# etrigger/Parsip

Hardware: AMD Instinct MI355X
Metric: Mcells/sec polygonized, 256^3 grid 32-prim BlobTree, at 1/2/4/8 MI355X (higher is better)
Workload: dtype f32

## Files before the change

### parsip_amd/csrc/psgpu_device.h

```cpp
#pragma once
#include "psgpu_model.h"

namespace psgpu {

typedef const __attribute__((address_space(4))) DevModel* ModelPtr;
typedef const __attribute__((address_space(4))) DevPrim CPrim;
typedef const __attribute__((address_space(4))) DevOp COp;
typedef const __attribute__((address_space(4))) CubeTablesDev* TablePtr;
__device__ __forceinline__ ModelPtr as_const(const DevModel* m) { return (ModelPtr)m; }
__device__ __forceinline__ TablePtr as_const(const CubeTablesDev* t) { return (TablePtr)t; }

__device__ __forceinline__ Instr load_instr(ModelPtr M, int pc) {
    typedef const __attribute__((address_space(4))) uint32_t* CU32;
    const CU32 w = (CU32)(&M->instr[pc]);
    const uint32_t words[3] = {w[0], w[1], w[2]};
    Instr I;
    __builtin_memcpy(&I, words, 12);
    return I;
}

__device__ __forceinline__ float max_ref(float a, float b) { return a > b ? a : b; }
__device__ __forceinline__ float min_ref(float a, float b) { return a < b ? a : b; }
__device__ __forceinline__ float m01(bool c) { return c ? 1.0f : 0.0f; }
__device__ __forceinline__ int lane_id() { return __lane_id(); }
// ... 210 lines not shown
    }
    return wyvill(prim_dist2<TYPE, PR>(P, x, y, z));
}

__device__ __forceinline__ float prim_field(CPrim& P, float pX, float pY, float pZ) {
    float x = pX, y = pY, z = pZ;
    if (P.hasMatrix) {
        x = ((P.mat[0] * pX + P.mat[1] * pY) + P.mat[2] * pZ) + P.mat[3];
        y = ((P.mat[4] * pX + P.mat[5] * pY) + P.mat[6] * pZ) + P.mat[7];
        z = ((P.mat[8] * pX + P.mat[9] * pY) + P.mat[10] * pZ) + P.mat[11];
    }
    float d2;
    switch (P.type) {
    case PSGPU_T_POINT: d2 = prim_dist2<PSGPU_T_POINT, CPrim>(P, x, y, z); break;
    case PSGPU_T_LINE: d2 = prim_dist2<PSGPU_T_LINE, CPrim>(P, x, y, z); break;
    case PSGPU_T_CYLINDER: d2 = prim_dist2<PSGPU_T_CYLINDER, CPrim>(P, x, y, z); break;
    case PSGPU_T_TRIANGLE: d2 = prim_dist2<PSGPU_T_TRIANGLE, CPrim>(P, x, y, z); break;
    case PSGPU_T_CUBE: d2 = prim_dist2<PSGPU_T_CUBE, CPrim>(P, x, y, z); break;
    case PSGPU_T_DISC: d2 = prim_dist2<PSGPU_T_DISC, CPrim>(P, x, y, z); break;
    case PSGPU_T_RING: d2 = prim_dist2<PSGPU_T_RING, CPrim>(P, x, y, z); break;
    default: d2 = 0.0f; break;
    }
    return wyvill(d2);
}

__device__ __forceinline__ float op_field(uint32_t type, float lf, float rf, float resY, float last) {
    switch (type) {
    case PSGPU_T_BLEND: return lf + rf;
    case PSGPU_T_RICCI: {
        const float base = lf + rf;
        float den = resY * base;
        den = resY - den;
        den = base + den;
        return base * (1.0f / den);
    }
    case PSGPU_T_UNION: return max_ref(lf, rf);
    case PSGPU_T_INTERSECT: return min_ref(lf, rf);
    case PSGPU_T_DIF: return min_ref(lf, 1.0f - rf);
    case PSGPU_T_SMOOTHDIF: return lf * (1.0f - rf);
    case 22: case 23: case 24: case 25: return lf;
    default: return last;
    }
}

__device__ __forceinline__ bool op_colour_weights(uint32_t type, float lf, float rf, float v, float* wl, float* wr) {
    switch (type) {
    case PSGPU_T_BLEND: case PSGPU_T_RICCI:
        *wl = 2.0f * (0.5f + lf) - 1.0f;
        *wr = 2.0f * (0.5f + rf) - 1.0f;
        return true;
    case PSGPU_T_UNION: case PSGPU_T_INTERSECT:
        *wl = m01((v - lf) == 0.0f);
        *wr = m01((v - rf) == 0.0f);
        return true;
    case PSGPU_T_DIF: case PSGPU_T_SMOOTHDIF:
        *wl = m01(lf == v);
        *wr = m01((1.0f - rf) == v);
        return true;
    default:
        return false;
    }
}

struct CullMask {
    uint64_t lo, hi;
    uint64_t inLo, inHi;
};
__device__ __forceinline__ bool op_inside(const CullMask& cm, uint32_t k) {
    return k < 64 ? ((cm.inLo >> k) & 1ull) : ((cm.inHi >> (k - 64)) & 1ull);
}

struct CullLanes {
    CullSeg s[2];
    bool two;
};

__device__ __forceinline__ CullSeg load_cullseg(ModelPtr M, int i) {
    typedef const __attribute__((address_space(4))) float* CF;
    const CF f = (CF)(&M->cull[i]);
    CullSeg S;
    S.a[0] = f[0]; S.a[1] = f[1]; S.a[2] = f[2];
    S.u[0] = f[3]; S.u[1] = f[4]; S.u[2] = f[5];
    S.invUU = f[6]; S.radius = f[7];
    S.tmin = f[8]; S.tmax = f[9]; S.axisClear = f[10]; S.pad = f[11];
    return S;
}

__device__ __forceinline__ CullLanes load_cull_lanes(ModelPtr M) {
    CullLanes L;
    L.two = M->ctPrims > 64u;
    L.s[0] = load_cullseg(M, lane_id());
    if (L.two) L.s[1] = load_cullseg(M, 64 + lane_id());
    return L;
}

__device__ __forceinline__ CullMask cull_mask_from(const CullLanes& L, float x0, float y0, float z0, float x1,
                                                   float y1, float z1) {
    CullMask cm{0ull, 0ull};
    float c[3], h;
    if (!cull_box(x0, y0, z0, x1, y1, z1, c, &h)) return cm;
    cm.lo = ballot(cull_one(L.s[0], c[0], c[1], c[2], h));
    if (L.two) cm.hi = ballot(cull_one(L.s[1], c[0], c[1], c[2], h));
    return cm;
}

__device__ __forceinline__ CullMask cull_mask_box(ModelPtr M, float x0, float y0, float z0, float x1, float y1,
                                                  float z1) {
    return cull_mask_from(load_cull_lanes(M), x0, y0, z0, x1, y1, z1);
}

__device__ __forceinline__ CullMask cull_mask_points(const CullLanes& L, float px, float py, float pz, bool enable,
                                                     float ext = 0.0f) {
    if (!enable) return CullMask{0ull, 0ull};
    if (ballot(!(px == px) || !(py == py) || !(pz == pz)) != 0ull) return CullMask{0ull, 0ull};
    return cull_mask_from(L, wave_min(px), wave_min(py), wave_min(pz), wave_max(px) + ext, wave_max(py) + ext,
                          wave_max(pz) + ext);
}
__device__ __forceinline__ CullMask cull_mask_points(ModelPtr M, float px, float py, float pz, bool enable,
                                                     float ext = 0.0f) {
    if (!enable) return CullMask{0ull, 0ull};
    return cull_mask_points(load_cull_lanes(M), px, py, pz, true, ext);
}

__device__ __forceinline__ bool culled(const CullMask& cm, uint32_t i) {
    return i < 64 ? ((cm.lo >> i) & 1ull) : ((cm.hi >> (i - 64)) & 1ull);
}

constexpr float kBoundEps = 2e-4f;

struct BoundBox {
    float cx, cy, cz, h;
    float xs[4], ys[4], zs[4];
};

template <int TYPE, class PR>
__device__ __forceinline__ float prim_true_dist(PR& P, float x, float y, float z, float* axisD) {
    float d2 = 0.0f;
    if (TYPE == PSGPU_T_POINT) {
        const float dx = x - P.pos[0], dy = y - P.pos[1], dz = z - P.pos[2];
        d2 = dx * dx + dy * dy + dz * dz;
    } else if (TYPE == PSGPU_T_LINE) {
        const float ux = P.dir[0] - P.pos[0], uy = P.dir[1] - P.pos[1], uz = P.dir[2] - P.pos[2];
        const float dx = x - P.pos[0], dy = y - P.pos[1], dz = z - P.pos[2];
        const float t = (dx * ux + dy * uy + dz * uz) / (ux * ux + uy * uy + uz * uz);
        const float ex = dx - t * ux, ey = dy - t * uy, ez = dz - t * uz;
        d2 = ex * ex + ey * ey + ez * ez;
    } else if (TYPE == PSGPU_T_CYLINDER) {
        const float px = x - P.pos[0], py = y - P.pos[1], pz = z - P.pos[2];
        float yy = px * P.dir[0] + py * P.dir[1] + pz * P.dir[2];
        const float rr = px * px + py * py + pz * pz - yy * yy;
        const float r = __builtin_amdgcn_sqrtf(rr > 0.0f ? rr : 0.0f);
        *axisD = r;
        const float xx = fmaxf(r - P.res[0], 0.0f);
        yy = yy > 0.0f ? fmaxf(yy - P.res[1], 0.0f) : yy;
        d2 = xx * xx + yy * yy;
    } else if (TYPE == PSGPU_T_CUBE) {
        const float ex = fmaxf(fabsf(x - P.pos[0]) - P.res[0], 0.0f);
        const float ey = fmaxf(fabsf(y - P.pos[1]) - P.res[0], 0.0f);
        const float ez = fmaxf(fabsf(z - P.pos[2]) - P.res[0], 0.0f);
        d2 = ex * ex + ey * ey + ez * ez;
    }
    return __builtin_amdgcn_sqrtf(d2);
}

__device__ __forceinline__ float wyvill_of_dist(float d) {
    const float t = 1.0f - d * d;
    return t > 0.0f ? (t * t) * t : 0.0f;
}

template <int TYPE, class PR>
__device__ __forceinline__ void prim_bound(PR& P, const BoundBox& B, float* lo, float* hi, bool* ok) {
    float axisD = 1e30f;
    const float d = prim_true_dist<TYPE, PR>(P, B.cx, B.cy, B.cz, &axisD);
    if (TYPE == PSGPU_T_CYLINDER) *ok = *ok && (axisD - B.h > 0.05f);
    *hi = wyvill_of_dist(fmaxf(d - B.h, 0.0f)) + kBoundEps;
    *lo = wyvill_of_dist(d + B.h) - kBoundEps;
}

__device__ __forceinline__ void bound_op(uint32_t type, float ll, float lh, float rl, float rh, float* lo, float* hi) {
    switch (type) {
    case PSGPU_T_BLEND: *lo = ll + rl; *hi = lh + rh; break;
    case PSGPU_T_UNION: *lo = fmaxf(ll, rl); *hi = fmaxf(lh, rh); break;
    case PSGPU_T_INTERSECT: *lo = fminf(ll, rl); *hi = fminf(lh, rh); break;
    case PSGPU_T_DIF: *lo = fminf(ll, 1.0f - rh); *hi = fminf(lh, 1.0f - rl); break;
    case PSGPU_T_SMOOTHDIF: {
        const float a = 1.0f - rh, b = 1.0f - rl;
        const float p0 = ll * a, p1 = ll * b, p2 = lh * a, p3 = lh * b;
        *lo = fminf(fminf(p0, p1), fminf(p2, p3));
        *hi = fmaxf(fmaxf(p0, p1), fmaxf(p2, p3));
    } break;
    default: *lo = ll; *hi = lh; break;
    }
}

template <class OR>
__device__ __forceinline__ void bound_prune(OR& b, const BoundBox& B, float* lo, float* hi) {
    bool anyZ = false, allX = true, noX = true, allY = true, noY = true;
#pragma unroll
    for (int i = 0; i < 4; ++i) {
        anyZ = anyZ | ((B.zs[i] >= b.lo[2]) & (b.hi[2] >= B.zs[i]));
        const bool ix = (B.xs[i] >= b.lo[0]) & (b.hi[0] >= B.xs[i]);
        const bool iy = (B.ys[i] >= b.lo[1]) & (b.hi[1] >= B.ys[i]);
        allX = allX & ix; noX = noX & !ix;
        allY = allY & iy; noY = noY & !iy;
    }
    if (!anyZ && noX && noY) {
        *lo = 0.0f;
        *hi = 0.0f;
    } else if (!(anyZ || allX || allY)) {
        *lo = fminf(*lo, 0.0f);
        *hi = fmaxf(*hi, 0.0f);
    }
}

struct InterpEval {
    ModelPtr M;
    float* sl;
    __device__ InterpEval(ModelPtr m, float* slots) : M(m), sl(slots) {}

    template <int GROUP, bool COLOR>
    __device__ __forceinline__ float eval(float px, float py, float pz, const CullMask& cm, float* colOut) const {
        const int n = (int)M->nInstr;
        const bool noOps = M->ctOps == 0;
        int resume = 0;
        float last = 0.0f, acc = 0.0f;
        float lc0 = 0.0f, lc1 = 0.0f, lc2 = 0.0f;
        constexpr int SW = COLOR ? 4 : 1;
        for (int pc = 0; pc < n; ++pc) {
            const Instr I = load_instr(M, pc);
            const bool act = pc >= resume;
            if (I.kind == kEnter) {
                COp& O = M->ops[I.idx];
                bool in = ((px >= O.lo[0]) & (O.hi[0] >= px)) | ((py >= O.lo[1]) & (O.hi[1] >= py)) |
                          ((pz >= O.lo[2]) & (O.hi[2] >= pz));
                bool anyIn = group_any<GROUP>(act && in);
                bool prune = act && !anyIn;
                if (prune) {
                    resume = I.skipTo;
                    sl[(I.out * SW) * 64] = 0.0f;
                    last = 0.0f;
                }
                if (!COLOR) {
                    if (ballot(pc + 1 >= resume) == 0ull) pc = I.skipTo - 1;
                }
            } else if (I.kind == kPrim) {
                if (COLOR) {
                    float f = 0.0f;
                    if (act && !culled(cm, I.idx)) f = prim_field(M->prims[I.idx], px, py, pz);
                    sl[(I.out * SW) * 64] = f;
                } else if (act) {
                    float f = 0.0f;
                    if (!culled(cm, I.idx)) f = prim_field(M->prims[I.idx], px, py, pz);
                    sl[I.out * 64] = f;
                }
            } else if (I.kind == kOp) {
                if (COLOR || act) {
                    const float lf = sl[(I.lslot * SW) * 64];
                    const float rf = sl[(I.rslot * SW) * 64];
                    float v = op_field(I.type, lf, rf, M->ops[I.idx].resY, last);
// ... 91 lines not shown
__device__ __forceinline__ void phase_stamp_after(const Params& p, int ph, uint32_t bit, float dep) {
    if (!PSGPU_FIN_PHASES || !(p.debug & bit) || !p.stamps) return;
    const uint32_t w = blockIdx.x * (blockDim.x >> 6) + (threadIdx.x >> 6);
    if (w >= p.stampCap) return;
    uint64_t t;
    asm volatile("s_memrealtime %0\n\ts_waitcnt lgkmcnt(0)" : "=s"(t) : "v"(dep));
    if (lane_id() == 0) p.stamps[3 * (size_t)kNumStampKernels * p.stampCap + 8 * (size_t)w + ph] = t;
}
__device__ __forceinline__ void span_end(const Params& p, int K, uint64_t t0) {
    const uint64_t t1 = stamp_now();
    if (lane_id() == 0) {
        uint64_t* s = p.spans + 2 * ((size_t)K * kSpanLanes + (blockIdx.x & (kSpanLanes - 1)));
        atomicMin(reinterpret_cast<unsigned long long*>(s), (unsigned long long)t0);
        atomicMax(reinterpret_cast<unsigned long long*>(s + 1), (unsigned long long)t1);
    }
}
__device__ __forceinline__ uint32_t wave_hw_id() {
    const uint32_t hw = (uint32_t)__builtin_amdgcn_s_getreg((31 << 11) | 4);
    const uint32_t xcc = (uint32_t)__builtin_amdgcn_s_getreg((31 << 11) | 20) & 15u;
    return (hw & 0xffffu) | (xcc << 16);
}
__device__ __forceinline__ void mpu_ticks_s1(const Params& p, uint32_t w, uint64_t t0) {
    uint64_t* r = p.mpuTicks + 4 * (size_t)w;
    r[0] = t0;
    r[1] = stamp_now();
    r[2] = 0ull;
    r[3] = (uint64_t)wave_hw_id();
}
__device__ __forceinline__ void mpu_ticks_s2(const Params& p, uint32_t m) {
    const uint64_t t = stamp_now();
    const uint32_t hw = wave_hw_id();
    if (lane_id() == 0) {
        uint64_t* r = p.mpuTicks + 4 * (size_t)(m - p.mpuBegin);
        atomicMax(reinterpret_cast<unsigned long long*>(r + 2), (unsigned long long)t);
        reinterpret_cast<uint32_t*>(r + 3)[1] = hw;
    }
}
#define PSGPU_STAMPED(K, ITEM, CALL)                                             \
    {                                                                             \
        const uint64_t t0_ = (p.stamps || p.spans) ? psgpu::stamp_now() : 0ull;  \
        uint32_t item_ = blockIdx.x * (blockDim.x >> 6) + (threadIdx.x >> 6);     \
        CALL;                                                                     \
        if (K == 1 && p.mpuTicks && ITEM != 0xffffffffu) psgpu::mpu_ticks_s2(p, ITEM); \
        if (p.stamps) psgpu::stamp_end(p, K, t0_, ITEM);                          \
        if (p.spans) psgpu::span_end(p, K, t0_);                                  \
    }

__device__ __forceinline__ void mpu_origin(const Params& p, uint32_t m, float o[3]) {
    uint32_t k, jk;
    const uint32_t i = div_by(m, p.dims[2] * p.dims[1], p.divMagic[1], &jk);
    const uint32_t j = div_by(jk, p.dims[2], p.divMagic[0], &k);
    o[0] = p.lo[0] + (float)i * p.side;
    o[1] = p.lo[1] + (float)j * p.side;
    o[2] = p.lo[2] + (float)k * p.side;
}

__device__ __forceinline__ uint32_t wave_sum(uint32_t v) { return lane_value(wave_incl_scan(v), 63); }


__device__ __forceinline__ uint32_t front_tag(const Params& p) { return p.ctr->epoch + 1u; }

__device__ __forceinline__ void stamp_live_word(const Params& p, bool on, const CullMask& cm, uint64_t above) {
    if (on && p.stamps && lane_id() == 0) {
        const uint32_t w = blockIdx.x * (blockDim.x >> 6) + (threadIdx.x >> 6);
        if (w < p.stampCap)
            p.stamps[3 * (size_t)kNumStampKernels * p.stampCap + 8 * (size_t)w + 7] =
                (uint64_t)(128 - __popcll(cm.lo) - __popcll(cm.hi)) | above;
    }
}

__device__ __forceinline__ BoundBox octant_box(const Params& p, const float o[3], int c) {
    BoundBox B;
#pragma unroll
    for (int i = 0; i < 4; ++i) {
        B.xs[i] = o[0] + (float)(4 * (c & 1) + i) * p.cs;
        B.ys[i] = o[1] + (float)(4 * ((c >> 1) & 1) + i) * p.cs;
        B.zs[i] = o[2] + (float)(4 * (c >> 2) + i) * p.cs;
    }
    const float hx = 0.5f * (B.xs[3] - B.xs[0]), hy = 0.5f * (B.ys[3] - B.ys[0]), hz = 0.5f * (B.zs[3] - B.zs[0]);
    B.cx = 0.5f * (B.xs[0] + B.xs[3]);
    B.cy = 0.5f * (B.ys[0] + B.ys[3]);
    B.cz = 0.5f * (B.zs[0] + B.zs[3]);
    B.h = __builtin_amdgcn_sqrtf(hx * hx + hy * hy + hz * hz) * 1.0001f + 1e-4f;
    return B;
}

__device__ __forceinline__ uint32_t proven_mask(bool ok, float lo, float hi, uint32_t flags8) {
    const uint64_t bOut = ballot(ok && hi < 0.5f), bIn = ballot(ok && lo >= 0.5f);
    uint32_t proven8 = 0;
#pragma unroll
    for (int q = 0; q < 8; ++q) {
        const bool all = ((bOut >> (8 * q)) & 0xffull) == 0xffull || ((bIn >> (8 * q)) & 0xffull) == 0xffull;
        proven8 |= (all ? 1u : 0u) << q;
    }
    return proven8 & flags8;
}

__device__ __forceinline__ CullMask queue_masks(const Params& p, const CullLanes& cl, const float o[3],
                                                uint32_t queue8, uint32_t mOf, int lane) {
    CullMask mine{0ull, 0ull};
    if (!p.cull) return mine;
    const float eg = 7.0f * p.cs + 0.001f;
    ModelPtr Mo = as_const(p.model);
    const uint32_t nOps = p.opInside ? Mo->ctOps : 0u;
    float bl[2][3], bh[2][3];
#pragma unroll
    for (int h = 0; h < 2; ++h) {
        const uint32_t k = 64u * h + (uint32_t)lane;
#pragma unroll
        for (int a = 0; a < 3; ++a) {
            bl[h][a] = k < nOps ? p.model->ops[k].lo[a] : 1.0f;
            bh[h][a] = k < nOps ? p.model->ops[k].hi[a] : -1.0f;
        }
    }
    for (uint32_t qm = queue8; qm != 0u; qm &= qm - 1u) {
        const int q = __builtin_ctz(qm);
        const float ox = __int_as_float(__builtin_amdgcn_readlane(__float_as_int(o[0]), 8 * q));
        const float oy = __int_as_float(__builtin_amdgcn_readlane(__float_as_int(o[1]), 8 * q));
        const float oz = __int_as_float(__builtin_amdgcn_readlane(__float_as_int(o[2]), 8 * q));
        CullMask g = cull_mask_from(cl, ox, oy, oz, ox + eg, oy + eg, oz + eg);
        if (nOps != 0u) g.inLo = ballot((uint32_t)lane < nOps && op_inside_box(bl[0], bh[0], ox, oy, oz, p.cs));
        if (nOps > 64u)
            g.inHi = ballot(64u + (uint32_t)lane < nOps && op_inside_box(bl[1], bh[1], ox, oy, oz, p.cs));
        const uint32_t wq = lane_value(mOf, q) - p.mpuBegin;
        if (lane == 0) {
            p.mpuMasks[4 * wq] = g.lo;
            p.mpuMasks[4 * wq + 1] = g.hi;
            p.mpuMasks[4 * wq + 2] = g.inLo;
            p.mpuMasks[4 * wq + 3] = g.inHi;
        }
        if (lane == q) mine = g;
    }
    return mine;
}

struct QueueEntry {
    uint32_t m;
    CullMask cm;

    template <bool FRONT, class T>
    static __device__ __forceinline__ void put(T* at, T v) {
        if constexpr (FRONT) __hip_atomic_store(at, v, __ATOMIC_RELAXED, __HIP_MEMORY_SCOPE_AGENT);
        else *at = v;
    }
    template <bool FRONT, class T>
    static __device__ __forceinline__ T get(T* at) {
        if constexpr (FRONT) return __hip_atomic_load(at, __ATOMIC_RELAXED, __HIP_MEMORY_SCOPE_AGENT);
        else return *at;
    }
    template <bool FRONT>
    __device__ __forceinline__ void store(const Params& p, uint32_t slotq) const {
        put<FRONT>(&p.pq[slotq], m);
        if (p.cull) {
            put<FRONT>(&p.pqMask[4 * slotq], cm.lo);
            put<FRONT>(&p.pqMask[4 * slotq + 1], cm.hi);
            put<FRONT>(&p.pqMask[4 * slotq + 2], cm.inLo);
            put<FRONT>(&p.pqMask[4 * slotq + 3], cm.inHi);
        }
    }
    static __device__ __forceinline__ void publish(const Params& p, uint32_t slotq, bool mine) {
        asm volatile("s_waitcnt vmcnt(0)" ::: "memory");
        if (mine) put<true>(&p.fqReady[slotq], front_tag(p));
    }
    template <bool FRONT>
    static __device__ __forceinline__ QueueEntry load(const Params& p, ModelPtr M, uint32_t slotq) {
        QueueEntry e{uniform(get<FRONT>(&p.pq[slotq])), CullMask{0ull, 0ull}};
// ... 1116 lines not shown
```

### parsip_amd/csrc/psgpu_host.cpp

```cpp
#include <hip/hip_runtime.h>

#include <atomic>
#include <algorithm>
#include <numeric>
#include <cmath>
#include <cstdio>
#include <cstdlib>
#include <cstring>
#include <ctime>
#include <functional>
#include <limits>
#include <memory>
#include <chrono>
#include <mutex>
#include <string>
#include <thread>
#include <vector>

#include "../../include/parsip_gpu.h"
#include "psgpu_internal.h"
#include "psgpu_launch.h"


using namespace psgpu;
// ... 186 lines not shown
        }
        D.nInstr = P.ctPrims;
        D.nSlots = 1;
    } else {
        ProgramBuilder b(O);
        b.emit(0, 0, 0);
        if (!b.ok) return PSGPU_RET_INVALID_BVH;
        D.nInstr = (uint32_t)b.prog.size();
        std::copy(b.prog.begin(), b.prog.end(), D.instr);
        D.nSlots = (uint32_t)std::max(1, b.maxSlot);
    }
    for (uint32_t i = 0; i < 128; ++i) {
        DevOp& d = D.ops[i];
        d.lo[0] = O.vBoxLoX[i]; d.lo[1] = O.vBoxLoY[i]; d.lo[2] = O.vBoxLoZ[i];
        d.hi[0] = O.vBoxHiX[i]; d.hi[1] = O.vBoxHiY[i]; d.hi[2] = O.vBoxHiZ[i];
        d.resY = O.resY[i];
        d.type = O.opType[i];
    }
    const float* pc[3] = {P.colorX, P.colorY, P.colorZ};
    std::function<void(int)> zero_col = [&](int op) {
        const uint32_t t = O.opType[op], kind = O.opChildKind[op];
        const uint32_t L = O.opLeftChild[op], R = O.opRightChild[op];
        if (kind & 2) zero_col((int)L);
        if (kind & 1) zero_col((int)R);
        float cl[3], cr[3];
        for (int k = 0; k < 3; ++k) {
            cl[k] = (kind & 2) ? D.zeroCol[L][k] : pc[k][L];
            cr[k] = (kind & 1) ? D.zeroCol[R][k] : pc[k][R];
        }
        const float lf = 0.0f, rf = 0.0f;
        float v = 0.0f, wl = 0.0f, wr = 0.0f;
        bool weighted = true;
        switch (t) {
        case PSGPU_OP_BLEND: v = lf + rf; wl = 2.0f * (0.5f + lf) - 1.0f; wr = 2.0f * (0.5f + rf) - 1.0f; break;
        case PSGPU_OP_UNION: v = lf > rf ? lf : rf; wl = (v - lf) == 0.0f ? 1.0f : 0.0f; wr = (v - rf) == 0.0f ? 1.0f : 0.0f; break;
        case PSGPU_OP_INTERSECT: v = lf < rf ? lf : rf; wl = (v - lf) == 0.0f ? 1.0f : 0.0f; wr = (v - rf) == 0.0f ? 1.0f : 0.0f; break;
        case PSGPU_OP_DIF: { const float q = 1.0f - rf; v = lf < q ? lf : q; wl = lf == v ? 1.0f : 0.0f; wr = (1.0f - rf) == v ? 1.0f : 0.0f; } break;
        case PSGPU_OP_SMOOTHDIF: v = lf * (1.0f - rf); wl = lf == v ? 1.0f : 0.0f; wr = (1.0f - rf) == v ? 1.0f : 0.0f; break;
        default: weighted = false; break;
        }
        for (int k = 0; k < 3; ++k) {
            if (weighted) D.zeroCol[op][k] = wl * cl[k] + wr * cr[k];
            else if (t >= PSGPU_OP_WARPTWIST && t <= PSGPU_OP_WARPSHEAR) D.zeroCol[op][k] = cl[k];
            else D.zeroCol[op][k] = 0.0f;
        }
    };
    if (O.ctOps > 0) zero_col(0);
    for (uint32_t i = 0; i < 128; ++i) {
        DevPrim& d = D.prims[i];
        d.pos[0] = P.posX[i]; d.pos[1] = P.posY[i]; d.pos[2] = P.posZ[i];
        d.dir[0] = P.dirX[i]; d.dir[1] = P.dirY[i]; d.dir[2] = P.dirZ[i];
        d.res[0] = P.resX[i]; d.res[1] = P.resY[i]; d.res[2] = P.resZ[i];
        d.col[0] = P.colorX[i]; d.col[1] = P.colorY[i]; d.col[2] = P.colorZ[i];
        d.type = P.skeletType[i];
        const uint32_t im = P.idxMatrix[i];
        d.hasMatrix = im != 0;
        if (im != 0) {
            if (im >= 128) return PSGPU_RET_PARAM_ERROR;
            memcpy(d.mat, &Mx.matrix[im * PSGPU_PRIM_MATRIX_STRIDE], 12 * sizeof(float));
        }
        bool c = !d.hasMatrix && finite3(d.pos);
        switch (d.type) {
        case PSGPU_PRIM_POINT: break;
        case PSGPU_PRIM_LINE: {
            const double ux = (double)d.dir[0] - d.pos[0], uy = (double)d.dir[1] - d.pos[1],
                         uz = (double)d.dir[2] - d.pos[2];
            c = c && finite3(d.dir) && (ux * ux + uy * uy + uz * uz) > 1e-6;
        } break;
        case PSGPU_PRIM_CUBE: c = c && std::isfinite(d.res[0]) && d.res[0] >= 0.0f; break;
        case PSGPU_PRIM_CYLINDER: {
            const double n2 = (double)d.dir[0] * d.dir[0] + (double)d.dir[1] * d.dir[1] + (double)d.dir[2] * d.dir[2];
            c = c && finite3(d.dir) && std::fabs(n2 - 1.0) < 1e-4 && d.res[0] >= 0.0f && d.res[1] >= 0.0f &&
                std::isfinite(d.res[0]) && std::isfinite(d.res[1]);
        } break;
        default: c = false; break;
        }
        CullSeg& cs = D.cull[i];
        memset(&cs, 0, sizeof(cs));
        const float inf = std::numeric_limits<float>::infinity();
        cs.radius = inf;
        cs.tmin = 0.0f;
        cs.tmax = 1.0f;
        cs.axisClear = -inf;
        uint32_t flags = c ? 1u : 0u;
        if (c) {
            for (int a = 0; a < 3; ++a) cs.a[a] = d.pos[a];
            cs.radius = 0.0f;
            double uu = 0.0;
            if (d.type == PSGPU_PRIM_LINE) {
                for (int a = 0; a < 3; ++a) cs.u[a] = d.dir[a] - d.pos[a];
                cs.tmin = -inf;
                cs.tmax = inf;
                flags |= 2u;
            } else if (d.type == PSGPU_PRIM_CYLINDER) {
                for (int a = 0; a < 3; ++a) cs.u[a] = d.res[1] * d.dir[a];
                cs.radius = d.res[0];
                cs.axisClear = 0.05f;
                flags |= 4u;
            } else if (d.type == PSGPU_PRIM_CUBE) {
                cs.radius = (float)(d.res[0] * 1.7320508075688772 * (1.0 + 1e-6));
            }
            for (int a = 0; a < 3; ++a) uu += (double)cs.u[a] * cs.u[a];
            cs.invUU = uu > 0.0 ? (float)(1.0 / uu) : 0.0f;
            if (d.type == PSGPU_PRIM_CYLINDER && uu == 0.0) {
                flags &= ~1u;
                cs.radius = inf;
            }
        } else if (d.type == PSGPU_PRIM_TRIANGLE) {
            cs.radius = -inf;
        }
        if (i >= P.ctPrims) cs.radius = inf;
        d.cullable = flags;
    }
    bool bnd = D.nInstr > 0;
    for (uint32_t k = 0; k < D.nInstr; ++k) {
        const Instr& I = D.instr[k];
        if (I.kind == kOp && !((I.type >= 14 && I.type <= 18) || (I.type >= 22 && I.type <= 25))) bnd = false;
        if (I.kind == kPrim || I.kind == kSumPrim) {
            const DevPrim& q = D.prims[I.idx];
            if (!(q.type == PSGPU_PRIM_TRIANGLE || (q.cullable & 1u))) bnd = false;
        }
    }
    D.boundable = bnd ? 1u : 0u;
    D.rootZeroValid = root_zero_set(D, D.rootZero) ? 1u : 0u;
    if (!D.rootZeroValid) D.rootZero[0] = D.rootZero[1] = 0ull;
    return PSGPU_RET_SUCCESS;
}

void lattice_dims(float cs, const PsVec3f& lo, const PsVec3f& hi, uint32_t d[3]) {
    const float ext[3] = {hi.x - lo.x, hi.y - lo.y, hi.z - lo.z};
    for (int a = 0; a < 3; ++a) {
        const float q = ext[a] / cs;
        const int cells = (int)std::ceil(q);
        int n = cells / PSGPU_CELLS_PER_MPU;
        if (cells % PSGPU_CELLS_PER_MPU != 0) ++n;
        d[a] = n > 0 ? (uint32_t)n : 0u;
    }
}

const char* kKernelNames[kNumKernels] = {"k_precheck", "k_mpu", "k_vertex", "k_finish"};

}

namespace psgpu {
int hip_fail(hipError_t e, const char* what) {
    if (e == hipSuccess) return PSGPU_RET_SUCCESS;
    fprintf(stderr, "psgpu: %s failed: %s\n", what, hipGetErrorString(e));
    return e == hipErrorOutOfMemory ? PSGPU_RET_NOT_ENOUGH_MEM : PSGPU_RET_DEVICE_ERROR;
}

int set_device(psgpu_ctx* c) { return hip_fail(hipSetDevice(c->device), "hipSetDevice"); }
}

namespace {

void brick_layout(const psgpu_ctx* c, uint32_t* i0, uint32_t bd[3]) {
    const uint32_t nyz = c->dims[1] * c->dims[2];
    const uint32_t first = nyz ? c->mpuBegin / nyz : 0;
    const uint32_t last = (nyz && c->mpuCount) ? (c->mpuBegin + c->mpuCount - 1) / nyz : first;
    *i0 = first / 2;
    bd[0] = c->mpuCount ? last / 2 - first / 2 + 1 : 0;
    bd[1] = (c->dims[1] + 1) / 2;
    bd[2] = (c->dims[2] + 1) / 2;
}
uint32_t brick_stride(uint32_t n, bool spread) {
    if (!spread || n < 3) return 1u;
    for (uint32_t s = (uint32_t)(n * 0.6180339887) | 1u; s > 1; --s)
        if (std::gcd(s, n) == 1u) return s;
    return 1u;
}
size_t brick_count(const psgpu_ctx* c) {
    uint32_t i0, bd[3];
    brick_layout(c, &i0, bd);
    return (size_t)bd[0] * bd[1] * bd[2];
}

uint32_t front_cap(size_t bricks) {
    const uint32_t b = (uint32_t)bricks;
    return std::max(front_sub_cap((b + 1u) / 2u, 2u), front_sub_cap((b + 3u) / 4u, 4u));
}

int ensure_buffers(psgpu_ctx* c, uint32_t mpuCount) {
    const size_t n = std::max<uint32_t>(mpuCount, 1);
    c->pShardCap = 8u * (uint32_t)((brick_count(c) + kShards - 1) / kShards);
    const size_t fq = 8 * front_cap(brick_count(c));
    const size_t nq = std::max<size_t>((size_t)c->pShardCap * kShards, fq);
    constexpr Growth H = Growth::ByHalf;
    PSGPU_CHECK(c->pq.reserve(nq, H));
    PSGPU_CHECK(c->pqMask.reserve(nq * 4, H));
    PSGPU_CHECK(c->liveList.reserve(brick_count(c), H));
    bool fresh = false;
    if (fq) PSGPU_CHECK(c->fqReady.reserve(fq, H, &fresh));
    if (fresh)
        PSGPU_CHECK(hipMemset(c->fqReady, 0, c->fqReady.cap * sizeof(uint32_t)));
// ... 1519 lines not shown
```

### parsip_amd/csrc/psgpu_model.h

```cpp
#pragma once
#ifdef __HIPCC_RTC__
typedef unsigned char uint8_t;
typedef signed char int8_t;
typedef unsigned short uint16_t;
typedef unsigned int uint32_t;
typedef int int32_t;
typedef unsigned long long uint64_t;
typedef long long int64_t;
#elif defined(PSGPU_MODEL_NO_HIP)
#include <stdint.h>
#else
#include <stdint.h>
#include <hip/hip_runtime.h>
#endif
#if defined(__HIPCC__) || defined(__HIPCC_RTC__)
#define PSGPU_HD __host__ __device__
#define PSGPU_HDI __host__ __device__ __forceinline__
#else
#define PSGPU_HD
#define PSGPU_HDI inline
#endif

namespace psgpu {

// ... 2 lines not shown
    const float mag = __builtin_fmaxf(__builtin_fabsf(o), __builtin_fabsf(hi));
    if (!(mag < 1e30f)) return false;
    const float m = 0.002f + 1e-5f * mag;
    return opLo <= o - m && hi + m <= opHi;
}
PSGPU_HD inline bool op_inside_box(const float opLo[3], const float opHi[3], float ox, float oy, float oz, float cs) {
    return op_inside_axis(opLo[0], opHi[0], ox, cs) || op_inside_axis(opLo[1], opHi[1], oy, cs) ||
           op_inside_axis(opLo[2], opHi[2], oz, cs);
}

#define PSGPU_T_CYLINDER 0
#define PSGPU_T_DISC 1
#define PSGPU_T_LINE 2
#define PSGPU_T_POINT 3
#define PSGPU_T_RING 4
#define PSGPU_T_CUBE 6
#define PSGPU_T_TRIANGLE 7
#define PSGPU_T_UNION 14
#define PSGPU_T_INTERSECT 15
#define PSGPU_T_DIF 16
#define PSGPU_T_SMOOTHDIF 17
#define PSGPU_T_BLEND 18
#define PSGPU_T_RICCI 19

struct CubeTablesDev {
    uint64_t row[256];
    uint64_t order[256];
    uint16_t cross[256];
    uint8_t ntri[256];
    uint16_t own[8];
    uint64_t edge;
    uint8_t pad[8];
    uint32_t crossNtri[256];
};

enum InstrKind : uint8_t { kEnter = 0, kPrim = 1, kOp = 2, kSumPrim = 3 };

struct Instr {
    uint8_t kind;
    uint8_t type;
    uint8_t out;
    uint8_t lslot;
    uint8_t rslot;
    uint8_t childKind;
    uint8_t L, R;
    uint16_t idx;
    uint16_t skipTo;
    uint32_t pad;
};
static_assert(sizeof(Instr) == 16, "Instr size");

struct DevOp {
    float lo[3];
    float hi[3];
    float resY;
    uint32_t type;
};
static_assert(sizeof(DevOp) == 32, "DevOp size");

struct DevPrim {
    float pos[3];
    float dir[3];
    float res[3];
    float col[3];
    uint32_t type;
    uint32_t hasMatrix;
    uint32_t cullable;
    float cullRadius;
    float mat[12];
    float pad[4];
};
static_assert(sizeof(DevPrim) == 128, "DevPrim size");

constexpr int kMaxInstr = 512;
constexpr int kMaxSlots = 64;

struct CullSeg {
    float a[3];
    float u[3];
    float invUU;
    float radius;
    float tmin, tmax;
    float axisClear;
    float pad;
};
static_assert(sizeof(CullSeg) == 48, "CullSeg size");

PSGPU_HDI float cull_sqrt(float x) {
#if defined(__HIP_DEVICE_COMPILE__)
    return __builtin_amdgcn_sqrtf(x);
#else
    return __builtin_sqrtf(x);
#endif
}

PSGPU_HDI bool cull_box(float x0, float y0, float z0, float x1, float y1, float z1, float c[3], float* h) {
    if (!(x1 - x0 < 1e30f && y1 - y0 < 1e30f && z1 - z0 < 1e30f)) return false;
    c[0] = 0.5f * (x0 + x1);
    c[1] = 0.5f * (y0 + y1);
    c[2] = 0.5f * (z0 + z1);
    const float hx = 0.5f * (x1 - x0), hy = 0.5f * (y1 - y0), hz = 0.5f * (z1 - z0);
    *h = cull_sqrt(hx * hx + hy * hy + hz * hz) * 1.0001f + 1e-6f;
    return true;
}

PSGPU_HDI bool cull_one(const CullSeg& S, float cx, float cy, float cz, float h) {
    const float dx = cx - S.a[0], dy = cy - S.a[1], dz = cz - S.a[2];
    const float t = (dx * S.u[0] + dy * S.u[1] + dz * S.u[2]) * S.invUU;
    const float lx = dx - t * S.u[0], ly = dy - t * S.u[1], lz = dz - t * S.u[2];
    const float lineDist = cull_sqrt(lx * lx + ly * ly + lz * lz);
    const float tc = __builtin_fminf(__builtin_fmaxf(t, S.tmin), S.tmax);
    const float ex = dx - tc * S.u[0], ey = dy - tc * S.u[1], ez = dz - tc * S.u[2];
    const float d = (cull_sqrt(ex * ex + ey * ey + ez * ez) - S.radius) - h;
    return d > 0.0f && d * d >= 1.02f && (lineDist - h > S.axisClear);
}

PSGPU_HDI void brick_box(const float lo[3], float side, const uint32_t dims[3], uint32_t bi, uint32_t bj,
                               uint32_t bk, float blo[3], float bhi[3]) {
    const uint32_t b[3] = {bi, bj, bk};
    for (int a = 0; a < 3; ++a) {
        const uint32_t m0 = 2u * b[a], last = dims[a] - 1u;
        const uint32_t i0 = m0 < last ? m0 : last, i1 = m0 + 1u < last ? m0 + 1u : last;
        blo[a] = lo[a] + (float)i0 * side;
        bhi[a] = side + (lo[a] + (float)i1 * side);
    }
}

PSGPU_HDI uint32_t div_by(uint32_t m, uint32_t d, uint32_t magic, uint32_t* rem) {
#if defined(__HIP_DEVICE_COMPILE__)
    uint32_t q = __umulhi(m, magic);
#else
    uint32_t q = (uint32_t)(((uint64_t)m * magic) >> 32);
#endif
    uint32_t r = m - q * d;
    if (r >= d) { ++q; r -= d; }
    if (r >= d) { ++q; r -= d; }
    *rem = r;
    return q;
}

struct DevModel {
    uint32_t nInstr;
    uint32_t nSlots;
    uint32_t ctPrims;
    uint32_t ctOps;
    uint32_t boundable;
    uint32_t pad[3];
    Instr instr[kMaxInstr];
    DevOp ops[128];
    DevPrim prims[128];
    CullSeg cull[128];
    float zeroCol[128][4];
    uint64_t rootZero[2];
    uint32_t rootZeroValid;
    uint32_t pad2;
};

#ifndef __HIPCC_RTC__
inline bool prim_maybe_culled(const DevPrim& P) {
    return P.type == PSGPU_T_TRIANGLE ||
           (!P.hasMatrix && (P.type == PSGPU_T_POINT || P.type == PSGPU_T_LINE || P.type == PSGPU_T_CYLINDER ||
                             P.type == PSGPU_T_CUBE));
}
inline bool zero_subtree_set(const DevModel& M, int op, uint64_t m[2], int depth = 0) {
    const Instr* I = nullptr;
    for (uint32_t k = 0; k < M.nInstr && !I; ++k)
        if (M.instr[k].kind == kOp && M.instr[k].idx == op) I = &M.instr[k];
    if (!I || depth > 128) return false;
    const int type = I->type, kind = I->childKind;
    auto child = [&](bool isOp, int id) {
        if (isOp) return zero_subtree_set(M, id, m, depth + 1);
        if (id >= 128 || !prim_maybe_culled(M.prims[id])) return false;
        m[id >> 6] |= 1ull << (id & 63);
        return true;
    };
    if (type >= 14 && type <= 18) return child((kind & 2) != 0, I->L) && child((kind & 1) != 0, I->R);
    if (type >= 22 && type <= 25) return child((kind & 2) != 0, I->L);
    return false;
}
inline bool root_zero_set(const DevModel& M, uint64_t m[2]) {
    m[0] = m[1] = 0ull;
    bool ok = true;
    if (M.ctOps == 0) {
        for (uint32_t k = 0; k < M.nInstr; ++k) {
            const uint32_t id = M.instr[k].idx;
            if (M.instr[k].kind != kSumPrim || id >= 128 || !prim_maybe_culled(M.prims[id])) return false;
            m[id >> 6] |= 1ull << (id & 63);
        }
        ok = M.nInstr > 0;
    } else {
        ok = zero_subtree_set(M, 0, m);
    }
    for (int i = 0; ok && i < 128; ++i)
        if (((m[i >> 6] >> (i & 63)) & 1ull) && !(M.cull[i].radius < __builtin_inff())) ok = false;
    return ok;
}
#endif
// ... 103 lines not shown
```

Before: 362,900.

## Tighten cull and field-interval bounds using per-axis box half extents

Replaces the bounding-sphere-radius tests in primitive culling and in per-octant field interval bounds with tighter per-axis tests. These use a support-function reach along the separation direction and an axis-aligned box gap, via a new boxHalf field in CullSeg. Tighter bounds should cull more primitives and prove more octants empty or full, so fewer cells need full field evaluation. In exchange each cull and bound test does more arithmetic (an extra rcp and sqrt). Loose extent padding is needed to keep the bounds conservative.

After: 372,100 (median of 6 runs). +2.5%, better.

```diff
diff --git a/parsip_amd/csrc/psgpu_device.h b/parsip_amd/csrc/psgpu_device.h
--- a/parsip_amd/csrc/psgpu_device.h
+++ b/parsip_amd/csrc/psgpu_device.h
@@ -316,7 +316,7 @@
     S.a[0] = f[0]; S.a[1] = f[1]; S.a[2] = f[2];
     S.u[0] = f[3]; S.u[1] = f[4]; S.u[2] = f[5];
     S.invUU = f[6]; S.radius = f[7];
-    S.tmin = f[8]; S.tmax = f[9]; S.axisClear = f[10]; S.pad = f[11];
+    S.tmin = f[8]; S.tmax = f[9]; S.axisClear = f[10]; S.boxHalf = f[11];
     return S;
 }
 
@@ -331,10 +331,10 @@
 __device__ __forceinline__ CullMask cull_mask_from(const CullLanes& L, float x0, float y0, float z0, float x1,
                                                    float y1, float z1) {
     CullMask cm{0ull, 0ull};
-    float c[3], h;
-    if (!cull_box(x0, y0, z0, x1, y1, z1, c, &h)) return cm;
-    cm.lo = ballot(cull_one(L.s[0], c[0], c[1], c[2], h));
-    if (L.two) cm.hi = ballot(cull_one(L.s[1], c[0], c[1], c[2], h));
+    float c[3], h, he[3];
+    if (!cull_box(x0, y0, z0, x1, y1, z1, c, &h, he)) return cm;
+    cm.lo = ballot(cull_one(L.s[0], c[0], c[1], c[2], h, he));
+    if (L.two) cm.hi = ballot(cull_one(L.s[1], c[0], c[1], c[2], h, he));
     return cm;
 }
 
@@ -360,55 +360,15 @@
     return i < 64 ? ((cm.lo >> i) & 1ull) : ((cm.hi >> (i - 64)) & 1ull);
 }
 
-constexpr float kBoundEps = 2e-4f;
-
 struct BoundBox {
     float cx, cy, cz, h;
+    float hx, hy, hz;
     float xs[4], ys[4], zs[4];
 };
 
 template <int TYPE, class PR>
-__device__ __forceinline__ float prim_true_dist(PR& P, float x, float y, float z, float* axisD) {
-    float d2 = 0.0f;
-    if (TYPE == PSGPU_T_POINT) {
-        const float dx = x - P.pos[0], dy = y - P.pos[1], dz = z - P.pos[2];
-        d2 = dx * dx + dy * dy + dz * dz;
-    } else if (TYPE == PSGPU_T_LINE) {
-        const float ux = P.dir[0] - P.pos[0], uy = P.dir[1] - P.pos[1], uz = P.dir[2] - P.pos[2];
-        const float dx = x - P.pos[0], dy = y - P.pos[1], dz = z - P.pos[2];
-        const float t = (dx * ux + dy * uy + dz * uz) / (ux * ux + uy * uy + uz * uz);
-        const float ex = dx - t * ux, ey = dy - t * uy, ez = dz - t * uz;
-        d2 = ex * ex + ey * ey + ez * ez;
-    } else if (TYPE == PSGPU_T_CYLINDER) {
-        const float px = x - P.pos[0], py = y - P.pos[1], pz = z - P.pos[2];
-        float yy = px * P.dir[0] + py * P.dir[1] + pz * P.dir[2];
-        const float rr = px * px + py * py + pz * pz - yy * yy;
-        const float r = __builtin_amdgcn_sqrtf(rr > 0.0f ? rr : 0.0f);
-        *axisD = r;
-        const float xx = fmaxf(r - P.res[0], 0.0f);
-        yy = yy > 0.0f ? fmaxf(yy - P.res[1], 0.0f) : yy;
-        d2 = xx * xx + yy * yy;
-    } else if (TYPE == PSGPU_T_CUBE) {
-        const float ex = fmaxf(fabsf(x - P.pos[0]) - P.res[0], 0.0f);
-        const float ey = fmaxf(fabsf(y - P.pos[1]) - P.res[0], 0.0f);
-        const float ez = fmaxf(fabsf(z - P.pos[2]) - P.res[0], 0.0f);
-        d2 = ex * ex + ey * ey + ez * ez;
-    }
-    return __builtin_amdgcn_sqrtf(d2);
-}
-
-__device__ __forceinline__ float wyvill_of_dist(float d) {
-    const float t = 1.0f - d * d;
-    return t > 0.0f ? (t * t) * t : 0.0f;
-}
-
-template <int TYPE, class PR>
 __device__ __forceinline__ void prim_bound(PR& P, const BoundBox& B, float* lo, float* hi, bool* ok) {
-    float axisD = 1e30f;
-    const float d = prim_true_dist<TYPE, PR>(P, B.cx, B.cy, B.cz, &axisD);
-    if (TYPE == PSGPU_T_CYLINDER) *ok = *ok && (axisD - B.h > 0.05f);
-    *hi = wyvill_of_dist(fmaxf(d - B.h, 0.0f)) + kBoundEps;
-    *lo = wyvill_of_dist(d + B.h) - kBoundEps;
+    prim_interval<TYPE, PR>(P, B.cx, B.cy, B.cz, B.h, B.hx, B.hy, B.hz, lo, hi, ok);
 }
 
 __device__ __forceinline__ void bound_op(uint32_t type, float ll, float lh, float rl, float rh, float* lo, float* hi) {
@@ -666,6 +626,11 @@
     B.cy = 0.5f * (B.ys[0] + B.ys[3]);
     B.cz = 0.5f * (B.zs[0] + B.zs[3]);
     B.h = __builtin_amdgcn_sqrtf(hx * hx + hy * hy + hz * hz) * 1.0001f + 1e-4f;
+    float mag = 0.0f;
+#pragma unroll
+    for (int a = 0; a < 3; ++a)
+        mag = fmaxf(mag, fmaxf(fabsf(p.lo[a]), fabsf(p.lo[a] + (float)p.dims[a] * p.side)));
+    B.hx = B.hy = B.hz = (1.5f * p.cs + 2.4e-7f * (mag + p.side)) * 1.0001f + 1e-4f;
     return B;
 }
 
diff --git a/parsip_amd/csrc/psgpu_host.cpp b/parsip_amd/csrc/psgpu_host.cpp
--- a/parsip_amd/csrc/psgpu_host.cpp
+++ b/parsip_amd/csrc/psgpu_host.cpp
@@ -292,6 +292,7 @@
         cs.tmin = 0.0f;
         cs.tmax = 1.0f;
         cs.axisClear = -inf;
+        cs.boxHalf = inf;
         uint32_t flags = c ? 1u : 0u;
         if (c) {
             for (int a = 0; a < 3; ++a) cs.a[a] = d.pos[a];
@@ -309,6 +310,9 @@
                 flags |= 4u;
             } else if (d.type == PSGPU_PRIM_CUBE) {
                 cs.radius = (float)(d.res[0] * 1.7320508075688772 * (1.0 + 1e-6));
+                cs.boxHalf = d.res[0];
+            } else {
+                cs.boxHalf = 0.0f;
             }
             for (int a = 0; a < 3; ++a) uu += (double)cs.u[a] * cs.u[a];
             cs.invUU = uu > 0.0 ? (float)(1.0 / uu) : 0.0f;
@@ -319,7 +323,10 @@
         } else if (d.type == PSGPU_PRIM_TRIANGLE) {
             cs.radius = -inf;
         }
-        if (i >= P.ctPrims) cs.radius = inf;
+        if (i >= P.ctPrims) {
+            cs.radius = inf;
+            cs.boxHalf = inf;
+        }
         d.cullable = flags;
     }
     bool bnd = D.nInstr > 0;
diff --git a/parsip_amd/csrc/psgpu_model.h b/parsip_amd/csrc/psgpu_model.h
--- a/parsip_amd/csrc/psgpu_model.h
+++ b/parsip_amd/csrc/psgpu_model.h
@@ -108,7 +108,7 @@
     float radius;
     float tmin, tmax;
     float axisClear;
-    float pad;
+    float boxHalf;
 };
 static_assert(sizeof(CullSeg) == 48, "CullSeg size");
 
@@ -128,6 +128,25 @@
     const float hx = 0.5f * (x1 - x0), hy = 0.5f * (y1 - y0), hz = 0.5f * (z1 - z0);
     *h = cull_sqrt(hx * hx + hy * hy + hz * hz) * 1.0001f + 1e-6f;
     return true;
+}
+
+PSGPU_HDI float box_half_extent(float x0, float x1, float c) { return 0.5f * (x1 - x0) + __builtin_fabsf(1.2e-7f * c); }
+
+PSGPU_HDI bool cull_box(float x0, float y0, float z0, float x1, float y1, float z1, float c[3], float* h,
+                        float e[3]) {
+    if (!cull_box(x0, y0, z0, x1, y1, z1, c, h)) return false;
+    e[0] = box_half_extent(x0, x1, c[0]) * 1.0001f + 1e-6f;
+    e[1] = box_half_extent(y0, y1, c[1]) * 1.0001f + 1e-6f;
+    e[2] = box_half_extent(z0, z1, c[2]) * 1.0001f + 1e-6f;
+    return true;
+}
+
+PSGPU_HDI float cull_rcp(float x) {
+#if defined(__HIP_DEVICE_COMPILE__)
+    return __builtin_amdgcn_rcpf(x);
+#else
+    return 1.0f / x;
+#endif
 }
 
 PSGPU_HDI bool cull_one(const CullSeg& S, float cx, float cy, float cz, float h) {
@@ -139,6 +158,90 @@
     const float ex = dx - tc * S.u[0], ey = dy - tc * S.u[1], ez = dz - tc * S.u[2];
     const float d = (cull_sqrt(ex * ex + ey * ey + ez * ez) - S.radius) - h;
     return d > 0.0f && d * d >= 1.02f && (lineDist - h > S.axisClear);
+}
+
+PSGPU_HDI bool cull_one(const CullSeg& S, float cx, float cy, float cz, float h, const float he[3]) {
+    const float dx = cx - S.a[0], dy = cy - S.a[1], dz = cz - S.a[2];
+    const float t = (dx * S.u[0] + dy * S.u[1] + dz * S.u[2]) * S.invUU;
+    const float lx = dx - t * S.u[0], ly = dy - t * S.u[1], lz = dz - t * S.u[2];
+    const float lineDist = cull_sqrt(lx * lx + ly * ly + lz * lz);
+    const float tc = __builtin_fminf(__builtin_fmaxf(t, S.tmin), S.tmax);
+    const float ex = dx - tc * S.u[0], ey = dy - tc * S.u[1], ez = dz - tc * S.u[2];
+    const float n = cull_sqrt(ex * ex + ey * ey + ez * ez);
+    const float sphere = (n - S.radius) - h;
+    const float reach = (he[0] * __builtin_fabsf(ex) + he[1] * __builtin_fabsf(ey) + he[2] * __builtin_fabsf(ez)) *
+                        cull_rcp(n);
+    const float support = (n - S.radius) - (reach * 1.0001f + 1e-6f);
+    const float gx = __builtin_fmaxf((__builtin_fabsf(dx) - he[0]) - S.boxHalf, 0.0f);
+    const float gy = __builtin_fmaxf((__builtin_fabsf(dy) - he[1]) - S.boxHalf, 0.0f);
+    const float gz = __builtin_fmaxf((__builtin_fabsf(dz) - he[2]) - S.boxHalf, 0.0f);
+    const float gap = cull_sqrt(gx * gx + gy * gy + gz * gz);
+    const float d = __builtin_fmaxf(__builtin_fmaxf(sphere, support), gap);
+    return d > 0.0f && d * d >= 1.02f && (lineDist - h > S.axisClear);
+}
+
+constexpr float kBoundEps = 2e-4f;
+
+template <int TYPE, class PR>
+PSGPU_HDI float prim_true_dist(PR& P, float x, float y, float z, float* axisD, float ev[3]) {
+    float d2 = 0.0f;
+    ev[0] = ev[1] = ev[2] = 0.0f;
+    if (TYPE == PSGPU_T_POINT) {
+        const float dx = x - P.pos[0], dy = y - P.pos[1], dz = z - P.pos[2];
+        ev[0] = __builtin_fabsf(dx); ev[1] = __builtin_fabsf(dy); ev[2] = __builtin_fabsf(dz);
+        d2 = dx * dx + dy * dy + dz * dz;
+    } else if (TYPE == PSGPU_T_LINE) {
+        const float ux = P.dir[0] - P.pos[0], uy = P.dir[1] - P.pos[1], uz = P.dir[2] - P.pos[2];
+        const float dx = x - P.pos[0], dy = y - P.pos[1], dz = z - P.pos[2];
+        const float t = (dx * ux + dy * uy + dz * uz) / (ux * ux + uy * uy + uz * uz);
+        const float ex = dx - t * ux, ey = dy - t * uy, ez = dz - t * uz;
+        ev[0] = __builtin_fabsf(ex); ev[1] = __builtin_fabsf(ey); ev[2] = __builtin_fabsf(ez);
+        d2 = ex * ex + ey * ey + ez * ez;
+    } else if (TYPE == PSGPU_T_CYLINDER) {
+        const float px = x - P.pos[0], py = y - P.pos[1], pz = z - P.pos[2];
+        float yy = px * P.dir[0] + py * P.dir[1] + pz * P.dir[2];
+        const float rr = px * px + py * py + pz * pz - yy * yy;
+        const float r = cull_sqrt(rr > 0.0f ? rr : 0.0f);
+        *axisD = r;
+        const float xx = __builtin_fmaxf(r - P.res[0], 0.0f);
+        const float k = xx > 0.0f ? xx * cull_rcp(r) : 0.0f;
+        const float ya = yy > 0.0f ? __builtin_fmaxf(yy - P.res[1], 0.0f) : yy;
+        ev[0] = __builtin_fabsf(k * (px - yy * P.dir[0]) + ya * P.dir[0]);
+        ev[1] = __builtin_fabsf(k * (py - yy * P.dir[1]) + ya * P.dir[1]);
+        ev[2] = __builtin_fabsf(k * (pz - yy * P.dir[2]) + ya * P.dir[2]);
+        d2 = xx * xx + ya * ya;
+    } else if (TYPE == PSGPU_T_CUBE) {
+        ev[0] = __builtin_fmaxf(__builtin_fabsf(x - P.pos[0]) - P.res[0], 0.0f);
+        ev[1] = __builtin_fmaxf(__builtin_fabsf(y - P.pos[1]) - P.res[0], 0.0f);
+        ev[2] = __builtin_fmaxf(__builtin_fabsf(z - P.pos[2]) - P.res[0], 0.0f);
+        d2 = ev[0] * ev[0] + ev[1] * ev[1] + ev[2] * ev[2];
+    }
+    return cull_sqrt(d2);
+}
+
+PSGPU_HDI float wyvill_of_dist(float d) {
+    const float t = 1.0f - d * d;
+    return t > 0.0f ? (t * t) * t : 0.0f;
+}
+
+template <int TYPE, class PR>
+PSGPU_HDI void prim_interval(PR& P, float cx, float cy, float cz, float h, float hx, float hy, float hz, float* lo,
+                             float* hi, bool* ok) {
+    float axisD = 1e30f, ev[3];
+    const float d = prim_true_dist<TYPE, PR>(P, cx, cy, cz, &axisD, ev);
+    if (TYPE == PSGPU_T_CYLINDER) *ok = *ok && (axisD - h > 0.05f);
+    const float reach = (hx * ev[0] + hy * ev[1] + hz * ev[2]) * cull_rcp(d);
+    float loD = __builtin_fmaxf(d - h, d - reach);
+    const float ux = ev[0] + hx, uy = ev[1] + hy, uz = ev[2] + hz;
+    const float hiD = __builtin_fminf(d + h, cull_sqrt(ux * ux + uy * uy + uz * uz));
+    if (TYPE == PSGPU_T_POINT || TYPE == PSGPU_T_CUBE) {
+        const float gx = __builtin_fmaxf(ev[0] - hx, 0.0f);
+        const float gy = __builtin_fmaxf(ev[1] - hy, 0.0f);
+        const float gz = __builtin_fmaxf(ev[2] - hz, 0.0f);
+        loD = __builtin_fmaxf(loD, cull_sqrt(gx * gx + gy * gy + gz * gz));
+    }
+    *hi = wyvill_of_dist(__builtin_fmaxf(loD, 0.0f)) + kBoundEps;
+    *lo = wyvill_of_dist(hiD) - kBoundEps;
 }
 
 PSGPU_HDI void brick_box(const float lo[3], float side, const uint32_t dims[3], uint32_t bi, uint32_t bj,
```
